# lucidrains/alphafold2

Hardware: NVIDIA B200
Metric: evoformer_residue_pairs_per_sec (higher is better)
Workload: dtype bf16

## Files before the change

### alphafold2_b200/_lib.py

```python
import ctypes as C
import os

_HERE = os.path.dirname(os.path.abspath(__file__))
LIB_PATH = os.environ.get("AF2_LIB_PATH") or os.path.join(_HERE, "csrc", "libaf2b200.so")

_lib = None

vp, ll, ci, cf = C.c_void_p, C.c_longlong, C.c_int, C.c_float


class FFWeights(C.Structure):
    _fields_ = [("ln_gamma", vp), ("ln_beta", vp), ("w1", vp), ("b1", vp), ("w2", vp), ("b2", vp), ("bn", ci),
                ("w_cat", vp), ("b_cat", vp), ("w_ext", vp)]


class AttnWeights(C.Structure):
    _fields_ = [("ln_gamma", vp), ("ln_beta", vp), ("w_qkv", vp), ("w_gate", vp), ("b_gate", vp),
                ("w_out", vp), ("b_out", vp), ("w_edge", vp), ("w_cat", vp), ("b_cat", vp), ("w_ext", vp)]


class TriMulWeights(C.Structure):
    _fields_ = [("ln_gamma", vp), ("ln_beta", vp), ("w_left", vp), ("b_left", vp), ("w_right", vp),
                ("b_right", vp), ("w_ogate", vp), ("b_ogate", vp), ("on_gamma", vp), ("on_beta", vp),
                ("w_out", vp), ("b_out", vp), ("bn", ci), ("w_cat", vp), ("b_cat", vp),
                ("w_ext", vp), ("w_ext_out", vp)]


class OuterWeights(C.Structure):
    _fields_ = [("ln_gamma", vp), ("ln_beta", vp), ("w_lr", vp), ("b_lr", vp), ("w_out", vp), ("b_out", vp),
                ("w_cat", vp), ("b_cat", vp), ("w_ext", vp), ("w_ext_out", vp)]


class FFWeightsStrict(C.Structure):
    _fields_ = [("ln_gamma", vp), ("ln_beta", vp), ("w1", vp), ("b1", vp), ("w2", vp), ("b2", vp)]


class AttnWeightsStrict(C.Structure):
    _fields_ = [("ln_gamma", vp), ("ln_beta", vp), ("w_qkvg", vp), ("b_qkvg", vp), ("w_out", vp), ("b_out", vp), ("w_edge", vp)]


class TriMulWeightsStrict(C.Structure):
    _fields_ = [("ln_gamma", vp), ("ln_beta", vp), ("w5", vp), ("b5", vp), ("on_gamma", vp), ("on_beta", vp),
                ("w_out", vp), ("b_out", vp)]


class OuterWeightsStrict(C.Structure):
    _fields_ = [("ln_gamma", vp), ("ln_beta", vp), ("w_lr", vp), ("b_lr", vp), ("w_out", vp), ("b_out", vp)]


_SIGNATURES = {
    "af2_last_error": (C.c_char_p, []),
    "af2_abi_version": (ci, []),
    "af2_check_device": (ci, []),
    "af2_set_proj_mode": (None, [ci]),
    "af2_debug_proj_trace": (ci, [C.POINTER(C.c_longlong)]),
    "af2_debug_attn_trace": (ci, [C.POINTER(C.c_longlong)]),
    "af2_launch_count": (C.c_ulonglong, []),
    "af2_profile_enable": (None, [ci]),
    "af2_profile_read": (ll, [ci, C.POINTER(C.c_double), C.POINTER(C.c_double), C.POINTER(C.c_double)]),
    "af2_feed_forward": (ci, [C.POINTER(FFWeights), vp, ll, ci, ci, vp, ll, vp]),
    "af2_feed_forward_workspace": (ll, [ll, ci, ci]),
    "af2_axial_attention": (ci, [C.POINTER(AttnWeights), vp, vp, vp, ci, ci, ci, ci, ci, ci, ci, vp, ll, vp]),
    "af2_axial_attention_ex": (ci, [C.POINTER(AttnWeights), vp, vp, vp, ci, ci, ci, ci, ci, ci, ci, ci, vp, ll, vp]),
    "af2_axial_attention_workspace": (ll, [ci, ci, ci, ci, ci, ci, ci]),
    "af2_triangle_multiply": (ci, [C.POINTER(TriMulWeights), vp, vp, ci, ci, ci, ci, vp, ll, vp]),
    "af2_triangle_multiply_workspace": (ll, [ci, ci, ci]),
    "af2_outer_mean": (ci, [C.POINTER(OuterWeights), vp, vp, vp, ci, ci, ci, ci, cf, vp, ll, vp]),
    "af2_outer_mean_workspace": (ll, [ci, ci, ci, ci]),
    "af2_pair_bias": (ci, [vp, vp, vp, ci, ci, ci, ci, vp]),
    "af2_axial_attention_prebias": (ci, [C.POINTER(AttnWeights), vp, vp, vp, ci, ci, ci, ci, ci, ci, ci, vp, ll, vp]),
    "af2_triangle_project": (ci, [C.POINTER(TriMulWeights), vp, vp, ll, ci, ci, vp, vp, ll, vp, vp, ll, vp]),
    "af2_triangle_project_workspace": (ll, [ll, ci]),
    "af2_triangle_contract": (ci, [C.POINTER(TriMulWeights), vp, vp, ll, vp, ll, ll, ci, vp, ci, ci, ci, ci, ci, vp, ll, vp]),
    "af2_triangle_contract_workspace": (ll, [ci, ci, ci]),
    "af2_outer_project": (ci, [C.POINTER(OuterWeights), vp, vp, ll, ci, ci, vp, ll, vp, ll, vp]),
    "af2_outer_project_workspace": (ll, [ll, ci]),
    "af2_outer_contract": (ci, [C.POINTER(OuterWeights), vp, vp, ll, vp, ll, ll, ci, vp, ci, ci, ci, ci, ci, cf, vp, ll, vp]),
    "af2_outer_contract_workspace": (ll, [ci, ci, ci]),
    "af2_rotary": (ci, [vp, vp, vp, vp, ci, ci, ci, ci, ci, ci, vp]),
    "af2_layernorm_bf16": (ci, [vp, vp, vp, vp, ll, ci, cf, vp]),
    "af2_gemm_bf16_f32": (ci, [vp, ll, ll, vp, ll, ll, vp, ll, ll, ci, ci, ci, ci, ci, vp]),
    "af2_feed_forward_strict": (ci, [C.POINTER(FFWeightsStrict), vp, ll, ci, ci, vp, ll, vp]),
    "af2_feed_forward_strict_workspace": (ll, [ll, ci, ci]),
    "af2_axial_attention_strict": (ci, [C.POINTER(AttnWeightsStrict), vp, vp, vp, ci, ci, ci, ci, ci, ci, ci, ci, vp, ll, vp]),
    "af2_axial_attention_strict_workspace": (ll, [ci, ci, ci, ci, ci, ci, ci]),
    "af2_triangle_multiply_strict": (ci, [C.POINTER(TriMulWeightsStrict), vp, vp, ci, ci, ci, ci, vp, ll, vp]),
    "af2_triangle_multiply_strict_workspace": (ll, [ci, ci, ci]),
    "af2_outer_mean_strict": (ci, [C.POINTER(OuterWeightsStrict), vp, vp, vp, ci, ci, ci, ci, cf, vp, ll, vp]),
    "af2_outer_mean_strict_workspace": (ll, [ci, ci, ci, ci]),
    "af2_embed_pair_init_workspace": (ll, [ci, ci, ci]),
    "af2_embed_pair_init": (ci, [vp, vp, vp, ci, vp, vp, vp, vp, vp, ci, vp, vp, vp, ci, ci, ci, ci, vp, ll, vp]),
    "af2_distogram_head": (ci, [vp, vp, vp, vp, vp, vp, ci, ci, ci, ci, vp]),
    "af2_l2_persist": (ci, [vp, ll, cf, vp]),
    "af2_split_bf16": (ci, [vp, vp, ll, ci, vp]),
    "af2_gemm_split_f32": (ci, [vp, vp, vp, ll, ci, ci, ci, ci, vp]),
    "af2_peer_ctrl_bytes": (ci, []),
    "af2_peer_can_access": (ci, [ci, ci]),
    "af2_peer_alloc": (ci, [ll, C.POINTER(vp)]),
    "af2_peer_free": (ci, [vp]),
    "af2_peer_export": (ci, [vp, vp]),
    "af2_peer_open": (ci, [vp, C.POINTER(vp)]),
    "af2_peer_close": (ci, [vp]),
    "af2_peer_error": (ci, [vp]),
    "af2_peer_exchange": (ci, [vp, ll, ll, vp, ll, ll, ci, ll, ci, ci, ci, vp]),
}

EXPORTED_SYMBOLS = tuple(_SIGNATURES)


def load():
    global _lib
    if _lib is None:
        if not os.path.isfile(LIB_PATH):
            raise RuntimeError(
                f"{LIB_PATH} not found: build it with `python -c 'import __graft_entry__ as g; g.build()'` "
                "(nvcc, sm_100a). alphafold2_b200 has no CPU or PyTorch fallback.")
        lib = C.CDLL(LIB_PATH)
        for name, (res, args) in _SIGNATURES.items():
            fn = getattr(lib, name)
            fn.restype = res
            fn.argtypes = args
        _lib = lib
    return _lib


def check(code: int):
    if code != 0:
        msg = load().af2_last_error().decode("utf-8", "replace")
        if code == -1:
            raise ValueError(f"af2b200: {msg}")
        raise RuntimeError(f"af2b200 (code {code}): {msg}")
```

### alphafold2_b200/csrc/api.cu

```cuda
#include <cuda.h>
#include <cuda_runtime.h>
#include <cudaTypedefs.h>
#include <nvtx3/nvToolsExt.h>

#include <cstdarg>
#include <cstdio>
#include <cstdlib>
#include <cstring>
#include <vector>

#include "../../include/af2b200.h"
#include "attention_tc.cuh"
#include "chan2tok_tma.cuh"
#include "gemm_tc.cuh"
#include "proj_tc.cuh"
#include "simt_kernels.cuh"
#include "strict_kernels.cuh"
#include "glue_kernels.cuh"

using namespace af2;

namespace {

thread_local char g_err[512] = "";

int fail(int code, const char* fmt, ...) {
  va_list ap;
  va_start(ap, fmt);
  vsnprintf(g_err, sizeof(g_err), fmt, ap);
  va_end(ap);
  return code;
}

#define CUDA_OK(expr)                                                                            \
  do {                                                                                           \
    cudaError_t _e = (expr);                                                                     \
    if (_e != cudaSuccess) return fail(AF2_ERR_CUDA, "%s: %s (%s:%d)", #expr, cudaGetErrorString(_e), __FILE__, __LINE__); \
  } while (0)
#define AF2_TRY(expr)            \
  do {                           \
    int _r = (expr);             \
    if (_r != AF2_OK) return _r; \
  } while (0)

constexpr int MAX_DEVICES = 64;
int cur_dev() {
  int dev = 0;
  cudaGetDevice(&dev);
  return (dev >= 0 && dev < MAX_DEVICES) ? dev : 0;
}
int sm_count() {
  static int n[MAX_DEVICES] = {0};
  const int dev = cur_dev();
  if (n[dev] == 0) {
    cudaDeviceGetAttribute(&n[dev], cudaDevAttrMultiProcessorCount, dev);
    if (n[dev] <= 0) n[dev] = 148;
  }
  return n[dev];
}

int g_x_evict_last = 0;
inline int x_hint(long long tokens, int d) {
  const double mb = (double)tokens * d * 4 / 1e6;
  return (g_x_evict_last && mb >= 48.0 && mb <= 100.0) ? 1 : 0;
}

int g_pdl = 1;
template <class... KArgs, class... Args>
cudaError_t launch_pdl(void (*kern)(KArgs...), dim3 grid, dim3 block, size_t smem, cudaStream_t s, Args&&... args) {
  cudaLaunchConfig_t cfg;
  memset(&cfg, 0, sizeof(cfg));
  cfg.gridDim = grid; cfg.blockDim = block; cfg.dynamicSmemBytes = smem; cfg.stream = s;
  cudaLaunchAttribute at[1];
  at[0].id = cudaLaunchAttributeProgrammaticStreamSerialization;
  at[0].val.programmaticStreamSerializationAllowed = 1;
  cfg.attrs = at; cfg.numAttrs = g_pdl ? 1 : 0;
  return cudaLaunchKernelEx(&cfg, kern, static_cast<KArgs>(args)...);
}

struct NvtxRange {
  explicit NvtxRange(const char* name) { nvtxRangePushA(name); }
  ~NvtxRange() { nvtxRangePop(); }
};

enum KClass { KC_GEMM_LINEAR = 0, KC_GEMM_CHANNEL = 1, KC_ATTENTION = 2, KC_LAYERNORM = 3, KC_CHAN2TOK = 4, KC_MISC = 5, KC_COUNT = 6 };
struct ProfRec { cudaEvent_t a, b; int cls; double flops, bytes; };
unsigned long long g_launches = 0;
bool g_prof = false;
std::vector<ProfRec> g_recs;
std::vector<cudaEvent_t> g_pool;

cudaEvent_t prof_event() {
  if (!g_pool.empty()) { cudaEvent_t e = g_pool.back(); g_pool.pop_back(); return e; }
  cudaEvent_t e; cudaEventCreate(&e); return e;
}
struct ProfScope {
  cudaStream_t s; bool on; ProfRec r;
// ... 390 lines not shown
  ProfScope ps(s, KC_CHAN2TOK, 0.0, (double)p.rows * p.n * p.d * (p.mode == 0 ? 8.0 : 6.0));
  chan_to_token_kernel<<<grid, 256, smem, s>>>(p);
  CUDA_OK(cudaGetLastError());
  return AF2_OK;
}

template <int DH>
int launch_attention_inst(const CUtensorMap& tq, const CUtensorMap& tk, const CUtensorMap& tv, const CUtensorMap& tbias,
                          const CUtensorMap& tg, const CUtensorMap& to, const AttnParams& p, cudaStream_t s) {
  using L = AttnSmem<DH>;
  static bool configured[MAX_DEVICES] = {false};
  auto kern = attention_tc_kernel<DH>;
  if (!configured[cur_dev()]) {
    CUDA_OK(cudaFuncSetAttribute(kern, cudaFuncAttributeMaxDynamicSharedMemorySize, L::TOTAL));
    configured[cur_dev()] = true;
  }
  const int nqb = (p.n + 127) / 128;
  const long long items = (long long)nqb * p.heads * p.nbatch;
  if (items <= 0) return AF2_OK;
  int grid = (int)(items < sm_count() ? items : sm_count());
  if (nqb >= 2 && nqb <= 8 && g_attn_group) grid = grid / nqb * nqb;
  const double tokens = (double)p.n * p.nbatch;
  ProfScope ps(s, KC_ATTENTION, 4.0 * tokens * p.n * p.heads * DH,
               tokens * p.heads * DH * 2.0 * 5 + (p.has_bias ? (double)p.heads * p.n * p.n * 2 : 0));
  CUDA_OK(launch_pdl(kern, dim3(grid), dim3(ATTN_THREADS), L::TOTAL, s, tq, tk, tv, tbias, tg, to, p));
  return AF2_OK;
}

int launch_attention(const __nv_bfloat16* qkv, int heads, int dh, int n, int nbatch, long long tok_sb, long long tok_si,
                     const __nv_bfloat16* bias, int npad, const uint8_t* mask, const __nv_bfloat16* gate,
                     __nv_bfloat16* out, cudaStream_t s, const __nv_bfloat16* qkv_hm = nullptr, long long hm_tokens = 0, int bias_t = 0) {
  const long long I = (long long)heads * dh;
  const long long ld = 3 * I;
  CUtensorMap tq, tk, tv, tb, tg, to;
  unsigned long long dims[4] = {(unsigned long long)dh, (unsigned long long)n, (unsigned long long)heads, (unsigned long long)nbatch};
  unsigned long long str[3] = {(unsigned long long)(tok_si * ld * 2), (unsigned long long)(dh * 2), (unsigned long long)(tok_sb * ld * 2)};
  if (qkv_hm) {
    str[0] = (unsigned long long)(tok_si * dh * 2); str[1] = (unsigned long long)(hm_tokens * dh * 2); str[2] = (unsigned long long)(tok_sb * dh * 2);
  }
  unsigned box[4] = {(unsigned)dh, 128, 1, 1};
  const CUtensorMapSwizzle swz = (dh == 64) ? CU_TENSOR_MAP_SWIZZLE_128B : CU_TENSOR_MAP_SWIZZLE_64B;
  const CUtensorMapL2promotion promo = (dh == 64) ? CU_TENSOR_MAP_L2_PROMOTION_L2_128B : CU_TENSOR_MAP_L2_PROMOTION_L2_64B;
  const CUtensorMapDataType bf = CU_TENSOR_MAP_DATA_TYPE_BFLOAT16;
  if (qkv_hm) {
    const long long part = (long long)heads * hm_tokens * dh;
    AF2_TRY(make_tmap(&tq, qkv_hm, 4, dims, str, box, swz, bf, CU_TENSOR_MAP_L2_PROMOTION_L2_256B));
    AF2_TRY(make_tmap(&tk, qkv_hm + part, 4, dims, str, box, swz, bf, CU_TENSOR_MAP_L2_PROMOTION_L2_256B));
    AF2_TRY(make_tmap(&tv, qkv_hm + 2 * part, 4, dims, str, box, swz, bf, CU_TENSOR_MAP_L2_PROMOTION_L2_256B));
  } else {
    AF2_TRY(make_tmap(&tq, qkv, 4, dims, str, box, swz, bf, promo));
    AF2_TRY(make_tmap(&tk, qkv + I, 4, dims, str, box, swz, bf, promo));
    AF2_TRY(make_tmap(&tv, qkv + 2 * I, 4, dims, str, box, swz, bf, promo));
  }
  unsigned long long gstr[3] = {(unsigned long long)(tok_si * I * 2), (unsigned long long)(dh * 2), (unsigned long long)(tok_sb * I * 2)};
  AF2_TRY(make_tmap(&tg, gate, 4, dims, gstr, box, swz, bf, promo));
  unsigned obox[4] = {(unsigned)dh, 32, 1, 1};
  AF2_TRY(make_tmap(&to, out, 4, dims, gstr, obox, swz));
  if (bias) {
    unsigned long long bd[3] = {(unsigned long long)npad, (unsigned long long)n, (unsigned long long)heads};
    unsigned long long bs[2] = {(unsigned long long)npad * 2, (unsigned long long)n * npad * 2};
    unsigned bb[3] = {64, 128, 1};
    AF2_TRY(make_tmap(&tb, bias, 3, bd, bs, bb, CU_TENSOR_MAP_SWIZZLE_128B));
  } else {
    tb = tq;
  }
  AttnParams p;
  memset(&p, 0, sizeof(p));
  p.n = n; p.heads = heads; p.nbatch = nbatch; p.has_bias = bias != nullptr;
  p.mask = mask; p.mask_sb = tok_sb; p.mask_si = tok_si;
  p.gate = gate; p.out = out; p.tok_sb = tok_sb; p.tok_si = tok_si; p.ld_gate = I; p.ld_out = I;
  p.l2_prefetch = g_attn_l2pf;
  p.k_stages3 = g_attn_k3;
  p.dbg_skip = g_attn_skip;
  p.ident_tmem = g_attn_ident_tmem;
  p.bias_t = bias_t;
  p.trace = g_attn_trace;
  if (dh == 64) return launch_attention_inst<64>(tq, tk, tv, tb, tg, to, p, s);
  if (dh == 32) return launch_attention_inst<32>(tq, tk, tv, tb, tg, to, p, s);
  return fail(AF2_ERR_BAD_ARG, "attention: dim_head %d unsupported (32 or 64)", dh);
}

#include "proj_launch.inl"

int launch_outer_scale(const uint8_t* mask, float* scale, uint32_t* words, int row0, int rows, int S, int N, float eps, cudaStream_t s);

int ew_grid(long long n) {
  long long b = (n + 255) / 256;
  long long cap = (long long)sm_count() * 8;
  return (int)(b < cap ? (b > 0 ? b : 1) : cap);
}

int launch_outer_scale(const uint8_t* mask, float* scale, uint32_t* words, int row0, int rows, int S, int N, float eps, cudaStream_t s) {
  const long long T = (long long)rows * N;
  if (T <= 0) return AF2_OK;
  const int nw = (S + 31) / 32;
  const size_t smem = (size_t)nw * N * 4;
  ProfScope ps(s, KC_MISC, 0.0, 0.0);
  if (words && smem <= 160 * 1024) {
    static size_t configured[MAX_DEVICES] = {0};
    if (smem > 48 * 1024 && smem > configured[cur_dev()]) {
      CUDA_OK(cudaFuncSetAttribute(outer_scale_bits_kernel, cudaFuncAttributeMaxDynamicSharedMemorySize, (int)smem));
      configured[cur_dev()] = smem;
    }
    mask_pack_bits_kernel<<<ew_grid((long long)nw * N), 256, 0, s>>>(mask, words, S, N);
    CUDA_OK(cudaGetLastError());
    const long long need = (T + 255) / 256;
    const int grid = (int)(need < sm_count() ? need : sm_count());
    outer_scale_bits_kernel<<<grid, 256, smem, s>>>(words, scale, row0, rows, S, N, eps);
  } else {
    outer_scale_rows_kernel<<<ew_grid(T), 256, 0, s>>>(mask, scale, row0, rows, S, N, eps);
  }
  CUDA_OK(cudaGetLastError());
  return AF2_OK;
}

}

extern "C" {

const char* af2_last_error(void) { return g_err; }
int af2_abi_version(void) { return 2; }

unsigned long long af2_launch_count(void) { return g_launches; }

void af2_profile_enable(int on) {
  g_prof = on != 0;
  if (g_prof) {
    for (auto& r : g_recs) { g_pool.push_back(r.a); g_pool.push_back(r.b); }
    g_recs.clear();
  }
}

long long af2_profile_read(int cls, double* ms, double* flops, double* bytes) {
  cudaDeviceSynchronize();
  double t = 0, f = 0, b = 0;
  long long n = 0;
  for (auto& r : g_recs) {
    if (r.cls != cls) continue;
    float e = 0.f;
    if (cudaEventElapsedTime(&e, r.a, r.b) == cudaSuccess) t += e;
    f += r.flops; b += r.bytes; ++n;
  }
  if (ms) *ms = t;
  if (flops) *flops = f;
  if (bytes) *bytes = b;
  return n;
}

int af2_debug_proj_trace(long long* out) {
  if (!g_proj_trace) return fail(AF2_ERR_BAD_ARG, "projection trace not enabled (AF2_PROJ_TRACE=1)");
  CUDA_OK(cudaDeviceSynchronize());
  CUDA_OK(cudaMemcpy(out, g_proj_trace, 2048 * sizeof(long long), cudaMemcpyDeviceToHost));
  return AF2_OK;
}

int af2_debug_attn_trace(long long* out) {
  if (!g_attn_trace) return fail(AF2_ERR_BAD_ARG, "attention trace not enabled (AF2_ATTN_TRACE=1)");
  CUDA_OK(cudaDeviceSynchronize());
  CUDA_OK(cudaMemcpy(out, g_attn_trace, 1024 * sizeof(long long), cudaMemcpyDeviceToHost));
  CUDA_OK(cudaMemset(g_attn_trace, 0, 1024 * sizeof(long long)));
  return AF2_OK;
}

void af2_set_proj_mode(int ctas) { g_proj_ctas = ctas < 0 ? 2 : (ctas > 2 ? 2 : ctas); }

int af2_check_device(void) {
  if (const char* e = getenv("AF2_PROJ_CTAS")) af2_set_proj_mode(atoi(e));
  if (const char* e = getenv("AF2_C2T_TMA")) g_c2t_tma = atoi(e) != 0;
  if (const char* e = getenv("AF2_PROJ_PRODTILES")) g_proj_prod_tiles = atof(e);
  if (const char* e = getenv("AF2_PROJ_BALANCE")) g_proj_balance = atoi(e) != 0;
  if (const char* e = getenv("AF2_PROJ_WIDE")) g_proj_wide = atoi(e) != 0;
  if (const char* e = getenv("AF2_PROJ_L2PF")) g_proj_l2pf = atoi(e) != 0;
  if (const char* e = getenv("AF2_GATHER_FUSED")) g_gather_fused = atoi(e) != 0;
  if (const char* e = getenv("AF2_ATTN_GROUP")) g_attn_group = atoi(e) != 0;
  if (const char* e = getenv("AF2_ATTN_L2PF")) g_attn_l2pf = atoi(e) != 0;
  if (const char* e = getenv("AF2_ATTN_HEADMAJOR")) g_attn_headmajor = atoi(e) != 0;
  if (const char* e = getenv("AF2_ATTN_K3")) g_attn_k3 = atoi(e) != 0;
  if (const char* e = getenv("AF2_ATTN_SKIP")) g_attn_skip = atoi(e);
  if (const char* e = getenv("AF2_ATTN_IDENT_TMEM")) g_attn_ident_tmem = atoi(e) != 0;
  if (const char* e = getenv("AF2_ATTN_BIAS_T")) g_attn_bias_t = atoi(e) != 0;
  if (const char* e = getenv("AF2_ATTN_TRACE")) {
    if (atoi(e) != 0 && !g_attn_trace) {
      if (cudaMalloc(&g_attn_trace, 1024 * sizeof(long long)) != cudaSuccess) g_attn_trace = nullptr;
      else cudaMemset(g_attn_trace, 0, 1024 * sizeof(long long));
    }
  }
  if (const char* e = getenv("AF2_X_EVICT_LAST")) g_x_evict_last = atoi(e) != 0;
  if (const char* e = getenv("AF2_PDL")) g_pdl = atoi(e) != 0;
  if (const char* e = getenv("AF2_PROJ_TRACE")) {
    if (atoi(e) != 0 && !g_proj_trace) {
      if (cudaMalloc(&g_proj_trace, 2048 * sizeof(long long)) != cudaSuccess) g_proj_trace = nullptr;
      else cudaMemset(g_proj_trace, 0, 2048 * sizeof(long long));
    }
  }
  int dev = 0;
  if (cudaGetDevice(&dev) != cudaSuccess) return fail(AF2_ERR_CUDA, "no CUDA device");
  int major = 0;
  cudaDeviceGetAttribute(&major, cudaDevAttrComputeCapabilityMajor, dev);
  if (major != 10) return fail(AF2_ERR_UNSUPPORTED_DEVICE, "libaf2b200 is built for sm_100a only; device has compute capability %d.x", major);
  return AF2_OK;
}

long long af2_feed_forward_workspace(long long tokens, int d, int hidden) {
  return align_up(tokens * d * 2, 256) + align_up(tokens * hidden * 2, 256) + 1024;
}

int af2_feed_forward(const af2_ff_weights* w, float* x, long long tokens, int d, int hidden, void* workspace,
                     long long workspace_bytes, af2_stream_t stream) {
  NvtxRange nvtx_("af2_feed_forward");
  cudaStream_t s = static_cast<cudaStream_t>(stream);
  if (!w || !x) return fail(AF2_ERR_BAD_ARG, "feed_forward: null argument");
  if (d % 8 || hidden % 8) return fail(AF2_ERR_BAD_ARG, "feed_forward: d=%d and hidden=%d must be multiples of 8", d, hidden);
  if (tokens > 0x7fffffffLL) return fail(AF2_ERR_BAD_ARG, "feed_forward: too many tokens");
  Arena ar(workspace, workspace_bytes);
  __nv_bfloat16* xn = ar.take<__nv_bfloat16>(tokens * d);
  __nv_bfloat16* hbuf = ar.take<__nv_bfloat16>(tokens * hidden);
  if (!ar.ok) return fail(AF2_ERR_WORKSPACE, "feed_forward: workspace too small");
  const int half = w->bn / 2;
  const int n1p = (hidden + half - 1) / half * w->bn;
  if (g_proj_ctas > 0 && w->w_cat && w->bn == 256 && proj_dim_ok(d)) {
    ProjCall pc;
    memset(&pc, 0, sizeof(pc));
    pc.x = x; pc.T = tokens; pc.d = d;
    pc.w_cat = w->w_cat; pc.w_ext = w->w_ext; pc.nseg = 1;
    pc.seg[0] = ProjOut{n1p / 256, EK_GATED_TOK_GELU, hidden, hbuf, hidden};
    AF2_TRY(launch_proj(pc, s));
  } else {
    LnParams lp;
    memset(&lp, 0, sizeof(lp));
    lp.x = x; lp.gamma = w->ln_gamma; lp.beta = w->ln_beta; lp.y = xn; lp.T = tokens; lp.d = d; lp.eps = 1e-5f;
    AF2_TRY(launch_layernorm(lp, s));
    GemmCall c1 = linear_call(xn, d, w->w1, d, (int)tokens, n1p, d);
    c1.bn = w->bn; c1.mode = EPI_GATED_BF16; c1.act = ACT_GELU; c1.layout = LAYOUT_TOKEN;
    c1.out = hbuf; c1.ld_out = hidden; c1.bias = w->b1; c1.out_cols = hidden;
    AF2_TRY(launch_gemm(c1, s));
  }
  GemmCall c2 = linear_call(hbuf, hidden, w->w2, hidden, (int)tokens, d, hidden);
  c2.mode = EPI_RESID_F32; c2.out = x; c2.ld_out = d; c2.bias = w->b2; c2.resid = x; c2.ld_resid = d;
  AF2_TRY(launch_gemm(c2, s));
  return AF2_OK;
}

long long af2_axial_attention_workspace(int B, int h, int wdim, int d, int heads, int dim_head, int row_attn) {
  const long long T = (long long)B * h * wdim, I = (long long)heads * dim_head;
  const int n = row_attn ? wdim : h;
  const long long npad = align_up(n, 8);
  return align_up(T * d * 2, 256) + 2 * align_up(T * 3 * I * 2, 256) + 2 * align_up(T * I * 2, 256) +
         align_up((long long)B * heads * n * npad * 2, 256) + 1024;
}

static int axial_attention_impl(const af2_attn_weights* w, float* x, const float* edges, const void* pre_bias,
                                const unsigned char* mask, int B, int h, int wdim, int d, int heads, int dim_head,
                                int row_attn, void* workspace, long long workspace_bytes, af2_stream_t stream, int tied = 0) {
  NvtxRange nvtx_(row_attn ? "af2_axial_attention(row)" : "af2_axial_attention(col)");
  cudaStream_t s = static_cast<cudaStream_t>(stream);
  if (!w || !x) return fail(AF2_ERR_BAD_ARG, "axial_attention: null argument");
  if (dim_head != 32 && dim_head != 64) return fail(AF2_ERR_BAD_ARG, "axial_attention: dim_head %d unsupported (32 or 64)", dim_head);
  if (d % 8) return fail(AF2_ERR_BAD_ARG, "axial_attention: dim %d must be a multiple of 8", d);
  const long long T = (long long)B * h * wdim, I = (long long)heads * dim_head;
  if (T > 0x7fffffffLL) return fail(AF2_ERR_BAD_ARG, "axial_attention: too many tokens");
  const int n = row_attn ? wdim : h;
  const int nb = row_attn ? h : wdim;
  const int npad = (int)align_up(n, 8);
  const bool has_bias = pre_bias != nullptr || (edges != nullptr && w->w_edge != nullptr);
  Arena ar(workspace, workspace_bytes);
  __nv_bfloat16* xn = ar.take<__nv_bfloat16>(T * d);
  __nv_bfloat16* qkv = ar.take<__nv_bfloat16>(T * 3 * I);
  __nv_bfloat16* gate = ar.take<__nv_bfloat16>(T * I);
  __nv_bfloat16* og = ar.take<__nv_bfloat16>(T * I);
  __nv_bfloat16* bias = ar.take<__nv_bfloat16>((long long)B * heads * n * npad);
  __nv_bfloat16* qkv_hm = ar.take<__nv_bfloat16>(T * 3 * I);
  if (!ar.ok) return fail(AF2_ERR_WORKSPACE, "axial_attention: workspace too small");
  if (pre_bias) bias = const_cast<__nv_bfloat16*>(static_cast<const __nv_bfloat16*>(pre_bias));

  const bool fused_proj = g_proj_ctas > 0 && w->w_cat && proj_dim_ok(d) && (I % 8) == 0;
  LnParams lp;
  memset(&lp, 0, sizeof(lp));
  lp.x = x; lp.gamma = w->ln_gamma; lp.beta = w->ln_beta; lp.y = xn; lp.T = T; lp.d = d; lp.eps = 1e-5f;
  const bool fuse_bias = has_bias && !pre_bias && edges == x && B == 1;
  const bool bias_t = g_attn_bias_t && has_bias && !pre_bias && pair_bias_fast_ok(d, heads) && !(fuse_bias && !fused_proj);
  if (has_bias && !pre_bias && npad != n) CUDA_OK(cudaMemsetAsync(bias, 0, (size_t)B * heads * n * npad * 2, s));
  if (fuse_bias) {
    lp.wb = w->w_edge; lp.bias_out = bias; lp.heads = heads; lp.bias_hs = (long long)n * npad; lp.n_inner = n; lp.pitch = npad;
  }
  if (!fused_proj) {
    AF2_TRY(launch_layernorm(lp, s));
  } else if (fuse_bias) {
    if (pair_bias_fast_ok(d, heads)) {
      AF2_TRY(launch_pair_bias(x, T, d, w->w_edge, bias, heads, (long long)n * npad, n, npad, s, bias_t ? 1 : 0));
    } else {
      lp.y = nullptr;
      AF2_TRY(launch_layernorm(lp, s));
    }
  }
  if (has_bias && !fuse_bias && !pre_bias && pair_bias_fast_ok(d, heads)) {
    for (int b = 0; b < B; ++b)
// ... 517 lines not shown
```

### include/af2b200.h

```cpp
#ifndef AF2B200_H
#define AF2B200_H
#ifdef __cplusplus
extern "C" {
#endif

typedef void* af2_stream_t;

#define AF2_OK 0
#define AF2_ERR_BAD_ARG (-1)
#define AF2_ERR_CUDA (-2)
#define AF2_ERR_UNSUPPORTED_DEVICE (-3)
#define AF2_ERR_WORKSPACE (-4)

const char* af2_last_error(void);
int af2_abi_version(void);
int af2_check_device(void);
void af2_set_proj_mode(int ctas);
int af2_debug_proj_trace(long long* out);
int af2_debug_attn_trace(long long* out);

unsigned long long af2_launch_count(void);
void af2_profile_enable(int on);
long long af2_profile_read(int cls, double* ms, double* flops, double* bytes);

typedef struct {
  const float* ln_gamma; const float* ln_beta;
  const void* w1; const float* b1;
  const void* w2; const float* b2;
  int bn;
  const void* w_cat; const float* b_cat;
  const void* w_ext;
} af2_ff_weights;
int af2_feed_forward(const af2_ff_weights* w, float* x, long long tokens, int d, int hidden,
                     void* workspace, long long workspace_bytes, af2_stream_t stream);
long long af2_feed_forward_workspace(long long tokens, int d, int hidden);

typedef struct {
  const float* ln_gamma; const float* ln_beta;
  const void* w_qkv;
  const void* w_gate; const float* b_gate;
  const void* w_out; const float* b_out;
  const float* w_edge;
  const void* w_cat; const float* b_cat;
  const void* w_ext;
} af2_attn_weights;
int af2_axial_attention(const af2_attn_weights* w, float* x, const float* edges, const unsigned char* mask,
                        int B, int h, int wdim, int d, int heads, int dim_head, int row_attn,
                        void* workspace, long long workspace_bytes, af2_stream_t stream);
int af2_axial_attention_ex(const af2_attn_weights* w, float* x, const float* edges, const unsigned char* mask, int B,
                           int h, int wdim, int d, int heads, int dim_head, int row_attn, int flags, void* workspace,
                           long long workspace_bytes, af2_stream_t stream);
long long af2_axial_attention_workspace(int B, int h, int wdim, int d, int heads, int dim_head, int row_attn);

typedef struct {
  const float* ln_gamma; const float* ln_beta;
  const void* w_left; const float* b_left;
  const void* w_right; const float* b_right;
  const void* w_ogate; const float* b_ogate;
  const float* on_gamma; const float* on_beta;
  const void* w_out; const float* b_out;
  int bn;
  const void* w_cat; const float* b_cat;
  const void* w_ext; const void* w_ext_out;
} af2_trimul_weights;
int af2_triangle_multiply(const af2_trimul_weights* w, float* x, const unsigned char* mask, int B, int N, int d,
                          int ingoing, void* workspace, long long workspace_bytes, af2_stream_t stream);
long long af2_triangle_multiply_workspace(int B, int N, int d);

typedef struct {
  const float* ln_gamma; const float* ln_beta;
  const void* w_lr; const float* b_lr;
  const void* w_out; const float* b_out;
  const void* w_cat; const float* b_cat;
  const void* w_ext; const void* w_ext_out;
} af2_outer_weights;
int af2_outer_mean(const af2_outer_weights* w, float* x, const float* m, const unsigned char* msa_mask,
                   int B, int S, int N, int d, float eps, void* workspace, long long workspace_bytes,
                   af2_stream_t stream);
long long af2_outer_mean_workspace(int B, int S, int N, int d);

int af2_pair_bias(const float* x_rows, const float* w_edge, void* bias_out, int rows, int n, int d, int heads,
                  af2_stream_t stream);
int af2_axial_attention_prebias(const af2_attn_weights* w, float* x, const void* bias_bf16, const unsigned char* mask,
                                int B, int h, int wdim, int d, int heads, int dim_head, int row_attn, void* workspace,
                                long long workspace_bytes, af2_stream_t stream);
int af2_triangle_project(const af2_trimul_weights* w, const float* x, const unsigned char* mask, long long tokens,
                         int inner, int d, void* Lc, void* Rc, long long chan_stride, void* gate, void* workspace,
                         long long workspace_bytes, af2_stream_t stream);
long long af2_triangle_project_workspace(long long tokens, int d);
int af2_triangle_contract(const af2_trimul_weights* w, float* x, const void* Lc, long long cs_l, const void* Rg,
                          long long cs_r, long long piece_stride, int pieces, const void* gate, int rows, int cols,
                          int K, int d, int ingoing, void* workspace, long long workspace_bytes, af2_stream_t stream);
long long af2_triangle_contract_workspace(int rows, int cols, int d);
int af2_outer_project(const af2_outer_weights* w, const float* m, const unsigned char* msa_mask, long long tokens,
                      int inner, int d, void* LRc, long long chan_stride, void* workspace, long long workspace_bytes,
                      af2_stream_t stream);
long long af2_outer_project_workspace(long long tokens, int d);
int af2_outer_contract(const af2_outer_weights* w, float* x, const void* Lc, long long cs_l, const void* Rg,
                       long long cs_r, long long piece_stride, int pieces, const unsigned char* msa_mask_full,
                       int row0, int rows, int N, int S, int d, float eps, void* workspace, long long workspace_bytes,
// ... 82 lines not shown
```

Measured before the change: 4.044 million.

## Fuse feed-forward LayerNorm, both GEMMs, GELU gating and residual into one kernel

Adds a persistent 2-CTA cluster tcgen05 kernel for the feed-forward block. It runs LayerNorm, the first projection with gated GELU, the second projection fed straight from tensor memory, then bias and residual add written back via TMA, all in one launch. This removes the bf16 hidden activation round-trip through global memory and the separate launches. The cost is a complex warp-specialised pipeline with many barriers, and it only applies to d of 128 or 256 with the cluster projection mode.

```diff
diff --git a/alphafold2_b200/_lib.py b/alphafold2_b200/_lib.py
--- a/alphafold2_b200/_lib.py
+++ b/alphafold2_b200/_lib.py
@@ -53,6 +53,7 @@
     "af2_abi_version": (ci, []),
     "af2_check_device": (ci, []),
     "af2_set_proj_mode": (None, [ci]),
+    "af2_set_ff_fused": (None, [ci]),
     "af2_debug_proj_trace": (ci, [C.POINTER(C.c_longlong)]),
     "af2_debug_attn_trace": (ci, [C.POINTER(C.c_longlong)]),
     "af2_launch_count": (C.c_ulonglong, []),
diff --git a/alphafold2_b200/csrc/api.cu b/alphafold2_b200/csrc/api.cu
--- a/alphafold2_b200/csrc/api.cu
+++ b/alphafold2_b200/csrc/api.cu
@@ -13,6 +13,7 @@
 #include "attention_tc.cuh"
 #include "chan2tok_tma.cuh"
 #include "gemm_tc.cuh"
+#include "ff_tc.cuh"
 #include "proj_tc.cuh"
 #include "simt_kernels.cuh"
 #include "strict_kernels.cuh"
@@ -569,6 +570,72 @@
 
 #include "proj_launch.inl"
 
+int g_ff_fused = 1;
+
+bool ff_fused_ok(const af2_ff_weights* w, int d, int hidden) {
+  return g_ff_fused && g_proj_ctas == 2 && w->w_cat && w->w_ext && w->bn == 256 && (d == 128 || d == 256) &&
+         hidden % FF_CHUNK == 0 && aligned16(w->w2) && aligned16(w->b2);
+}
+
+int launch_ff_fused(const af2_ff_weights* w, float* x, long long T, int d, int hidden, cudaStream_t s) {
+  if (T <= 0) return AF2_OK;
+  if (!aligned16(x)) return fail(AF2_ERR_BAD_ARG, "feed_forward: x not 16-byte aligned");
+  using L = FfSmem;
+  static bool configured_dev[MAX_DEVICES] = {false};
+  static int max_clusters_dev[MAX_DEVICES] = {0};
+  int& max_clusters = max_clusters_dev[cur_dev()];
+  if (!configured_dev[cur_dev()]) {
+    CUDA_OK(cudaFuncSetAttribute(ff_tc_kernel, cudaFuncAttributeMaxDynamicSharedMemorySize, L::TOTAL));
+    cudaLaunchConfig_t qc;
+    memset(&qc, 0, sizeof(qc));
+    qc.gridDim = dim3(sm_count(), 1, 1); qc.blockDim = dim3(FF_THREADS, 1, 1); qc.dynamicSmemBytes = L::TOTAL;
+    cudaLaunchAttribute qa[1];
+    qa[0].id = cudaLaunchAttributeClusterDimension; qa[0].val.clusterDim.x = 2; qa[0].val.clusterDim.y = 1; qa[0].val.clusterDim.z = 1;
+    qc.attrs = qa; qc.numAttrs = 1;
+    int nc = 0;
+    if (cudaOccupancyMaxActiveClusters(&nc, ff_tc_kernel, &qc) != cudaSuccess || nc <= 0) { cudaGetLastError(); nc = sm_count() / 2; }
+    max_clusters = nc < sm_count() / 2 ? nc : sm_count() / 2;
+    configured_dev[cur_dev()] = true;
+  }
+  const int n1p = (hidden + 127) / 128 * 256;
+  CUtensorMap tw1, tb1, tw2, tx;
+  {
+    unsigned long long dw[2] = {(unsigned long long)d, (unsigned long long)n1p};
+    unsigned long long sw[1] = {(unsigned long long)d * 2};
+    unsigned bw[2] = {64, 64};
+    AF2_TRY(make_tmap(&tw1, w->w_cat, 2, dw, sw, bw, CU_TENSOR_MAP_SWIZZLE_128B));
+    unsigned long long dx[2] = {16ull, (unsigned long long)n1p};
+    unsigned long long sx[1] = {32ull};
+    unsigned bx[2] = {16, 64};
+    AF2_TRY(make_tmap(&tb1, w->w_ext, 2, dx, sx, bx, CU_TENSOR_MAP_SWIZZLE_32B));
+    unsigned long long d2[2] = {(unsigned long long)hidden, (unsigned long long)d};
+    unsigned long long s2[1] = {(unsigned long long)hidden * 2};
+    unsigned b2[2] = {64, (unsigned)(d / 2)};
+    AF2_TRY(make_tmap(&tw2, w->w2, 2, d2, s2, b2, CU_TENSOR_MAP_SWIZZLE_128B));
+    unsigned long long dxr[2] = {(unsigned long long)d, (unsigned long long)T};
+    unsigned long long sxr[1] = {(unsigned long long)d * 4};
+    unsigned bxr[2] = {32, 32};
+    AF2_TRY(make_tmap(&tx, x, 2, dxr, sxr, bxr, CU_TENSOR_MAP_SWIZZLE_128B, CU_TENSOR_MAP_DATA_TYPE_FLOAT32));
+  }
+  FfParams p;
+  memset(&p, 0, sizeof(p));
+  p.x = x; p.b2 = w->b2; p.T = T; p.d = d; p.hidden = hidden; p.inv_d = 1.0f / (float)d; p.eps = 1e-5f;
+  p.m_units = (int)((T + 255) / 256);
+  const int clusters = p.m_units < max_clusters ? p.m_units : max_clusters;
+  const double flops = 2.0 * T * (double)d * hidden * 3;
+  const double bytes = (double)T * d * 8 + (double)n1p * d * 2 + (double)d * hidden * 2;
+  ProfScope ps(s, KC_GEMM_LINEAR, flops, bytes);
+  cudaLaunchConfig_t cfg;
+  memset(&cfg, 0, sizeof(cfg));
+  cfg.gridDim = dim3(clusters * 2, 1, 1); cfg.blockDim = dim3(FF_THREADS, 1, 1); cfg.dynamicSmemBytes = L::TOTAL; cfg.stream = s;
+  cudaLaunchAttribute at[2];
+  at[0].id = cudaLaunchAttributeClusterDimension; at[0].val.clusterDim.x = 2; at[0].val.clusterDim.y = 1; at[0].val.clusterDim.z = 1;
+  at[1].id = cudaLaunchAttributeProgrammaticStreamSerialization; at[1].val.programmaticStreamSerializationAllowed = 1;
+  cfg.attrs = at; cfg.numAttrs = g_pdl ? 2 : 1;
+  CUDA_OK(cudaLaunchKernelEx(&cfg, ff_tc_kernel, tw1, tb1, tw2, tx, p));
+  return AF2_OK;
+}
+
 int launch_outer_scale(const uint8_t* mask, float* scale, uint32_t* words, int row0, int rows, int S, int N, float eps, cudaStream_t s);
 
 int ew_grid(long long n) {
@@ -650,9 +717,11 @@
 }
 
 void af2_set_proj_mode(int ctas) { g_proj_ctas = ctas < 0 ? 2 : (ctas > 2 ? 2 : ctas); }
+void af2_set_ff_fused(int on) { g_ff_fused = on != 0; }
 
 int af2_check_device(void) {
   if (const char* e = getenv("AF2_PROJ_CTAS")) af2_set_proj_mode(atoi(e));
+  if (const char* e = getenv("AF2_FF_FUSED")) af2_set_ff_fused(atoi(e));
   if (const char* e = getenv("AF2_C2T_TMA")) g_c2t_tma = atoi(e) != 0;
   if (const char* e = getenv("AF2_PROJ_PRODTILES")) g_proj_prod_tiles = atof(e);
   if (const char* e = getenv("AF2_PROJ_BALANCE")) g_proj_balance = atoi(e) != 0;
@@ -699,6 +768,7 @@
   if (!w || !x) return fail(AF2_ERR_BAD_ARG, "feed_forward: null argument");
   if (d % 8 || hidden % 8) return fail(AF2_ERR_BAD_ARG, "feed_forward: d=%d and hidden=%d must be multiples of 8", d, hidden);
   if (tokens > 0x7fffffffLL) return fail(AF2_ERR_BAD_ARG, "feed_forward: too many tokens");
+  if (ff_fused_ok(w, d, hidden)) return launch_ff_fused(w, x, tokens, d, hidden, s);
   Arena ar(workspace, workspace_bytes);
   __nv_bfloat16* xn = ar.take<__nv_bfloat16>(tokens * d);
   __nv_bfloat16* hbuf = ar.take<__nv_bfloat16>(tokens * hidden);
diff --git a/alphafold2_b200/csrc/ff_tc.cuh b/alphafold2_b200/csrc/ff_tc.cuh
--- /dev/null
+++ b/alphafold2_b200/csrc/ff_tc.cuh
@@ -0,0 +1,314 @@
+#pragma once
+#include "proj_tc.cuh"
+
+namespace af2 {
+
+constexpr int FF_THREADS = 512;
+constexpr int FF_CHUNK = 64;
+
+struct FfParams {
+  float* x;
+  const float* b2;
+  long long T;
+  int d, hidden;
+  float inv_d, eps;
+  int m_units;
+};
+
+struct FfSmem {
+  static constexpr int STAGES = 5;
+  static constexpr int STAGE = 16384;
+  static constexpr int A_OFF = 0;
+  static constexpr int W_OFF = 2 * PROJ_A_BUF;
+  static constexpr int BIAS_OFF = W_OFF + STAGES * STAGE;
+  static constexpr int BIAS_BYTES = 64 * 32;
+  static constexpr int AEXT_OFF = BIAS_OFF + 2 * BIAS_BYTES;
+  static constexpr int BAR_OFF = AEXT_OFF + 256;
+  static constexpr int TOTAL = BAR_OFF + 512;
+  static_assert(TOTAL <= 232448, "exceeds the 227 KB of shared memory a CTA can use");
+};
+
+__device__ __forceinline__ void umma_bf16_ts_pair(uint32_t d_tmem, uint32_t a_tmem, uint64_t bdesc, uint32_t idesc,
+                                                  uint32_t accumulate) {
+  asm volatile(
+      "{\n\t.reg .pred p;\n\t"
+      "setp.ne.b32 p, %4, 0;\n\t"
+      "tcgen05.mma.cta_group::2.kind::f16 [%0], [%1], %2, %3, p;\n\t}"
+      ::"r"(d_tmem), "r"(a_tmem), "l"(bdesc), "r"(idesc), "r"(accumulate)
+      : "memory");
+}
+
+__global__ void __launch_bounds__(FF_THREADS, 1)
+ff_tc_kernel(const __grid_constant__ CUtensorMap tmW1, const __grid_constant__ CUtensorMap tmB1,
+             const __grid_constant__ CUtensorMap tmW2, const __grid_constant__ CUtensorMap tmX,
+             const __grid_constant__ FfParams p) {
+  using L = FfSmem;
+  constexpr int STAGES = L::STAGES;
+  extern __shared__ __align__(1024) uint8_t smem[];
+  if ((smem_u32(smem) & 1023u) != 0) __trap();
+  uint64_t* full_bar = reinterpret_cast<uint64_t*>(smem + L::BAR_OFF);
+  uint64_t* empty_bar = full_bar + STAGES;
+  uint64_t* bfull_bar = empty_bar + STAGES;
+  uint64_t* bempty_bar = bfull_bar + 2;
+  uint64_t* c1full_bar = bempty_bar + 2;
+  uint64_t* hfull_bar = c1full_bar + 2;
+  uint64_t* afull_bar = hfull_bar + 2;
+  uint64_t* aempty_bar = afull_bar + 2;
+  uint64_t* ofull_bar = aempty_bar + 2;
+  uint64_t* oempty_bar = ofull_bar + 1;
+  uint64_t* res_bar = oempty_bar + 1;
+  uint32_t* tmem_slot = reinterpret_cast<uint32_t*>(res_bar + 16);
+
+  const int warp = threadIdx.x >> 5;
+  const int lane = threadIdx.x & 31;
+  const uint32_t rank = cluster_ctarank();
+  const bool is_leader = rank == 0;
+  const int cluster_id = blockIdx.x / 2;
+  const int nclusters = gridDim.x / 2;
+  constexpr uint32_t TMEM_COLS = 512;
+  constexpr uint32_t ACC1_COL = 256;
+
+  if (warp == 0 && lane == 0) {
+    prefetch_tmap(&tmW1);
+    prefetch_tmap(&tmB1);
+    prefetch_tmap(&tmW2);
+    prefetch_tmap(&tmX);
+  }
+  if (warp == 1 && lane == 0) {
+    for (int s = 0; s < STAGES; ++s) {
+      mbar_init(&full_bar[s], 1);
+      mbar_init(&empty_bar[s], 1);
+    }
+    for (int s = 0; s < 2; ++s) {
+      mbar_init(&bfull_bar[s], 1);
+      mbar_init(&bempty_bar[s], 1);
+      mbar_init(&c1full_bar[s], 1);
+      mbar_init(&hfull_bar[s], 16);
+      mbar_init(&afull_bar[s], 2 * PROJ_NPROD);
+      mbar_init(&aempty_bar[s], 8);
+    }
+    mbar_init(ofull_bar, 1);
+    mbar_init(oempty_bar, 16);
+    for (int s = 0; s < 16; ++s) mbar_init(&res_bar[s], 1);
+    fence_barrier_init();
+  }
+  if (warp == 2) tmem_alloc_pair(tmem_slot, TMEM_COLS);
+  for (int i = threadIdx.x; i < 256 / 16; i += FF_THREADS)
+    *reinterpret_cast<uint4*>(smem + L::AEXT_OFF + i * 16) = make_uint4(0x3f803f80u, 0u, 0u, 0u);
+  fence_proxy_async_smem();
+  tc_fence_before();
+  cluster_sync_all();
+  tc_fence_after();
+  const uint32_t tmem_base = *tmem_slot;
+  pdl_launch_dependents();
+  pdl_wait();
+
+  const int my_units = p.m_units > cluster_id ? (p.m_units - 1 - cluster_id) / nclusters + 1 : 0;
+  const int nch = p.hidden / FF_CHUNK;
+  const int nchunks = my_units * nch;
+  const int nkb = p.d / GEMM_BK;
+  const int d_half = p.d >> 1;
+  auto unit_of = [&](int it) { return cluster_id + it * nclusters; };
+
+  if (warp == 0) {
+    if (lane == 0) {
+      auto leader_bar = [&](uint64_t* bar) { return mapa_u32(smem_u32(bar), 0); };
+      int stage = 0;
+      uint32_t phase = 0;
+      auto acquire = [&](int bytes) {
+        mbar_wait(&empty_bar[stage], phase ^ 1);
+        if (is_leader) mbar_arrive_expect_tx(&full_bar[stage], 2 * bytes);
+        return smem + L::W_OFF + stage * L::STAGE;
+      };
+      auto advance = [&]() { if (++stage == STAGES) { stage = 0; phase ^= 1; } };
+      auto load_w1 = [&](int g) {
+        const int c = g % nch;
+        const int row0 = (c >> 1) * 256 + static_cast<int>(rank) * 128 + (c & 1) * 64;
+        const int b = g & 1;
+        mbar_wait(&bempty_bar[b], ((g >> 1) & 1) ^ 1);
+        if (is_leader) mbar_arrive_expect_tx(&bfull_bar[b], 2 * L::BIAS_BYTES);
+        tma_load_2d_pair(smem + L::BIAS_OFF + b * L::BIAS_BYTES, &tmB1, leader_bar(&bfull_bar[b]), 0, row0);
+        for (int kb = 0; kb < nkb; kb += 2) {
+          uint8_t* sb = acquire(2 * 8192);
+          tma_load_2d_pair(sb, &tmW1, leader_bar(&full_bar[stage]), kb * GEMM_BK, row0);
+          tma_load_2d_pair(sb + 8192, &tmW1, leader_bar(&full_bar[stage]), (kb + 1) * GEMM_BK, row0);
+          advance();
+        }
+      };
+      auto load_w2 = [&](int g) {
+        const int c = g % nch;
+        uint8_t* sb = acquire(d_half * 128);
+        tma_load_2d_pair(sb, &tmW2, leader_bar(&full_bar[stage]), c * FF_CHUNK, static_cast<int>(rank) * d_half);
+        advance();
+      };
+      if (nchunks > 0) load_w1(0);
+      for (int g = 0; g < nchunks; ++g) {
+        if (g + 1 < nchunks) load_w1(g + 1);
+        load_w2(g);
+      }
+    }
+  } else if (warp == 1) {
+    if (is_leader) {
+      const uint32_t idesc1 = umma_idesc_bf16(256, 128, 0, 0);
+      const uint32_t idesc2 = umma_idesc_bf16(256, p.d, 0, 0);
+      int stage = 0;
+      uint32_t phase = 0;
+      auto ff1 = [&](int g) {
+        const int it = g / nch, c = g - it * nch;
+        const int ab = it & 1;
+        if (c == 0) mbar_wait(&afull_bar[ab], (it >> 1) & 1);
+        const int b = g & 1;
+        const uint32_t d_tmem = tmem_base + ACC1_COL + b * 128;
+        mbar_wait(&bfull_bar[b], (g >> 1) & 1);
+        tc_fence_after();
+        if (elect_one()) {
+          const uint64_t adesc = umma_smem_desc(smem_u32(smem + L::AEXT_OFF), 16, 0, SWZ_32);
+          const uint64_t bdesc = umma_smem_desc(smem_u32(smem + L::BIAS_OFF + b * L::BIAS_BYTES), 16, 256, SWZ_32);
+          umma_bf16_pair(d_tmem, adesc, bdesc, idesc1, 0u);
+          umma_commit_pair(&bempty_bar[b], 3);
+        }
+        __syncwarp();
+        const uint32_t sa0 = smem_u32(smem + L::A_OFF + ab * PROJ_A_BUF);
+        for (int kb = 0; kb < nkb; kb += 2) {
+          mbar_wait(&full_bar[stage], phase);
+          tc_fence_after();
+          if (elect_one()) {
+            const uint32_t sb = smem_u32(smem + L::W_OFF + stage * L::STAGE);
+#pragma unroll
+            for (int h = 0; h < 2; ++h) {
+#pragma unroll
+              for (int k = 0; k < GEMM_BK / 16; ++k) {
+                const uint64_t adesc = umma_smem_desc(sa0 + (kb + h) * 16384 + k * 32, 16, 1024, SWZ_128);
+                const uint64_t bdesc = umma_smem_desc(sb + h * 8192 + k * 32, 16, 1024, SWZ_128);
+                umma_bf16_pair(d_tmem, adesc, bdesc, idesc1, 1u);
+              }
+            }
+            umma_commit_pair(&empty_bar[stage], 3);
+            if (kb + 2 >= nkb) {
+              umma_commit_pair(&c1full_bar[b], 3);
+            }
+          }
+          __syncwarp();
+          if (++stage == STAGES) { stage = 0; phase ^= 1; }
+        }
+      };
+      auto ff2 = [&](int g) {
+        const int it = g / nch, c = g - it * nch;
+        const int b = g & 1;
+        mbar_wait(&hfull_bar[b], (g >> 1) & 1);
+        if (c == 0) mbar_wait(oempty_bar, (it & 1) ^ 1);
+        mbar_wait(&full_bar[stage], phase);
+        tc_fence_after();
+        if (elect_one()) {
+          const uint32_t sb = smem_u32(smem + L::W_OFF + stage * L::STAGE);
+          const uint32_t a_tmem = tmem_base + ACC1_COL + b * 128;
+#pragma unroll
+          for (int k = 0; k < FF_CHUNK / 16; ++k) {
+            const uint64_t bdesc = umma_smem_desc(sb + k * 32, 16, 1024, SWZ_128);
+            umma_bf16_ts_pair(tmem_base, a_tmem + (k >> 1) * 32 + (k & 1) * 8, bdesc, idesc2, (c != 0 || k != 0) ? 1u : 0u);
+          }
+          umma_commit_pair(&empty_bar[stage], 3);
+          if (c == nch - 1) umma_commit_pair(ofull_bar, 3);
+        }
+        __syncwarp();
+        if (++stage == STAGES) { stage = 0; phase ^= 1; }
+      };
+      if (nchunks > 0) ff1(0);
+      for (int g = 0; g < nchunks; ++g) {
+        if (g + 1 < nchunks) ff1(g + 1);
+        ff2(g);
+      }
+    }
+  } else if (warp >= 4 && warp < 12) {
+    const int q = warp & 3;
+    const int grp = (warp - 4) >> 2;
+    const uint32_t lane_sel = static_cast<uint32_t>(q * 32) << 16;
+    const uint32_t oempty_remote = mapa_u32(smem_u32(oempty_bar), 0);
+    const int ncc = p.d >> 6;
+    int g = 0;
+    uint32_t rc = 0;
+    for (int it = 0; it < my_units; ++it) {
+      for (int c = 0; c < nch; ++c, ++g) {
+        const int b = g & 1;
+        mbar_wait(&c1full_bar[b], (g >> 1) & 1);
+        tc_fence_after();
+        const uint32_t t_acc = tmem_base + lane_sel + ACC1_COL + b * 128 + grp * 32;
+        uint32_t u[32], gt[32], pk[16];
+        tmem_ld32(t_acc, u);
+        tmem_ld32(t_acc + 64, gt);
+        tmem_ld_wait();
+        proj_finish32<EK_GATED_TOK_GELU>(u, gt, 1.0f, pk);
+        tmem_st16(t_acc, pk);
+        tmem_st_wait();
+        tc_fence_before();
+        __syncwarp();
+        if (lane == 0) mbar_arrive_cluster(mapa_u32(smem_u32(&hfull_bar[b]), 0));
+      }
+      const int m0w = (unit_of(it) * 2 + static_cast<int>(rank)) * 128 + q * 32;
+      uint8_t* wbuf = smem + L::A_OFF + (it & 1) * PROJ_A_BUF + (warp - 4) * 8192;
+      uint64_t* rbar = res_bar + (warp - 4) * 2;
+      auto load_res = [&](int j) {
+        mbar_arrive_expect_tx(&rbar[j & 1], 4096);
+        tma_load_2d(wbuf + (j & 1) * 4096, &tmX, &rbar[j & 1], (grp + 2 * j) * 32, m0w);
+      };
+      mbar_wait(ofull_bar, it & 1);
+      tc_fence_after();
+      if (lane == 0) {
+        load_res(0);
+        if (ncc > 1) load_res(1);
+      }
+#pragma unroll 1
+      for (int j = 0; j < ncc; ++j, ++rc) {
+        const int col = (grp + 2 * j) * 32;
+        uint32_t v[32];
+        tmem_ld32(tmem_base + lane_sel + col, v);
+        tmem_ld_wait();
+        if (j == ncc - 1) {
+          tc_fence_before();
+          __syncwarp();
+          if (lane == 0) mbar_arrive_cluster(oempty_remote);
+        }
+        mbar_wait(&rbar[j & 1], (rc >> 1) & 1);
+        uint8_t* eb = wbuf + (j & 1) * 4096;
+        const float4* bias = reinterpret_cast<const float4*>(p.b2 + col);
+#pragma unroll
+        for (int e = 0; e < 8; ++e) {
+          float4* sp = reinterpret_cast<float4*>(eb + swz128_off(lane, e));
+          const float4 r4 = *sp, b4 = __ldg(bias + e);
+          *sp = make_float4(__uint_as_float(v[4 * e]) + b4.x + r4.x, __uint_as_float(v[4 * e + 1]) + b4.y + r4.y,
+                            __uint_as_float(v[4 * e + 2]) + b4.z + r4.z, __uint_as_float(v[4 * e + 3]) + b4.w + r4.w);
+        }
+        fence_proxy_async_smem();
+        __syncwarp();
+        if (lane == 0) {
+          tma_store_2d(&tmX, eb, col, m0w);
+          tma_store_commit();
+          if (j + 2 < ncc) {
+            tma_store_wait_read<0>();
+            load_res(j + 2);
+          }
+        }
+      }
+      if (lane == 0) {
+        tma_store_wait_read<0>();
+        mbar_arrive(&aempty_bar[it & 1]);
+      }
+      __syncwarp();
+    }
+  } else if (warp >= 12) {
+    const int pi = warp - 12;
+    auto item_row0 = [&](int it) { return static_cast<long long>(unit_of(it) * 2 + static_cast<int>(rank)) * 128; };
+    auto wait_empty = [&](int it) { mbar_wait(&aempty_bar[it & 1], ((it >> 1) & 1) ^ 1); };
+    auto signal_full = [&](int it) { mbar_arrive_cluster(mapa_u32(smem_u32(&afull_bar[it & 1]), 0)); };
+    uint8_t* a_base = smem + L::A_OFF;
+    if (p.d == 256) proj_producer_loop<8, PROJ_NPROD>(p.x, p.T, p.d, p.inv_d, p.eps, a_base, my_units, pi, lane, item_row0, wait_empty, signal_full, false, false);
+    else proj_producer_loop<4, PROJ_NPROD>(p.x, p.T, p.d, p.inv_d, p.eps, a_base, my_units, pi, lane, item_row0, wait_empty, signal_full, false, false);
+  }
+
+  __syncwarp();
+  tc_fence_before();
+  cluster_sync_all();
+  if (warp == 2) tmem_dealloc_pair(tmem_base, TMEM_COLS);
+}
+
+}
diff --git a/include/af2b200.h b/include/af2b200.h
--- a/include/af2b200.h
+++ b/include/af2b200.h
@@ -16,6 +16,7 @@
 int af2_abi_version(void);
 int af2_check_device(void);
 void af2_set_proj_mode(int ctas);
+void af2_set_ff_fused(int on);
 int af2_debug_proj_trace(long long* out);
 int af2_debug_attn_trace(long long* out);
 
```

Measured after the change: 4.235 million (median of 6 runs). 1.05x the previous value.
